# rlorenzo/facet

Hardware: AMD Instinct MI355X
Metric: images/sec whole-node (TOPIQ+SAMP+CLIP+InsightFace ensemble), 1024² batch (higher is better)
Workload: dtype f32

## Files before the change

### facet_amd/csrc/engine.hip

```cpp
#include "engine.h"
#include "onnx_graph.h"
#include "wino64_maps.h"
#include <algorithm>
#include <cmath>
#include <cstdlib>

namespace fe {

void WeightStore::set(const std::string& name, const float* data, const int64_t* shape, int ndim) {
  HostTensor h;
  h.shape.assign(shape, shape + ndim);
  h.data.assign(data, data + h.numel());
  t_[name] = std::move(h);
}
const HostTensor& WeightStore::get(const std::string& name) const {
  auto it = t_.find(name);
  if (it == t_.end()) throw Error("missing weight tensor '" + name + "'");
  return it->second;
}

float* DeviceWeights::upload(const std::vector<float>& v) {
  void* p = nullptr;
  const size_t b = v.size() * sizeof(float);
  FE_HIP(hipMalloc(&p, b ? b : 16));
// ... 219 lines not shown
  p.w = w.w; p.scale = w.scale; p.shift = w.shift; p.slope = w.slope;
  FE_CHECK(o.act != ACT_PRELU || w.slope, "conv: PReLU without slopes");
  if (o.res) {
    FE_CHECK(o.res->c == y.c && o.res->pixels() == y.pixels(), "conv: residual shape mismatch");
    p.res = o.res->p; p.ldr = o.res->ld;
  }
  if (o.gate) {
    FE_CHECK(o.gate->pixels() == y.pixels() && (o.gate->c == 1 || o.gate->c == y.c), "conv: gate shape mismatch");
    p.gate = o.gate->p; p.ldg = o.gate->ld; p.gate_c1 = o.gate->c == 1;
  }
  p.y = y.p; p.ldy = y.ld;
  p.N = x.n; p.H = x.h; p.W = x.w; p.Cin = w.CinPad;
  p.Ho = y.h; p.Wo = y.w; p.Cout = w.Cout;
  p.KH = w.KH; p.KW = w.KW; p.sh = o.sh; p.sw = o.sw; p.ph = o.ph; p.pw = o.pw; p.dh = o.dh; p.dw = o.dw;
  FE_CHECK(y.h == conv_out_dim(x.h, w.KH, o.sh, o.ph, o.dh) && y.w == conv_out_dim(x.w, w.KW, o.sw, o.pw, o.dw),
           "conv: output dims %dx%d inconsistent with input %dx%d", y.h, y.w, x.h, x.w);
  p.K = w.K; p.Kp = w.Kp;
  p.M = (int)y.pixels();
  FE_CHECK(y.pixels() < (1ull << 31), "conv: M too large");
  p.act = o.act; p.res_after_act = o.res_after_act;
  p.variant = c.force_variant;
  if (w.wtap && o.act != ACT_PRELU && o.sh == 1 && o.sw == 1 && !o.res && !o.gate && p.variant == 0 && y.h == x.h && y.w == x.w) {
    const int T = w.KH * w.KW * w.Cout, Tp = (T + 3) & ~3;
    const size_t mark = c.arena.mark();
    Tensor z = c.arena.tensor(x.n, x.h, x.w, Tp);
    ConvParams q{};
    q.x = x.p; q.ldx = x.ld; q.w = w.wtap; q.y = z.p; q.ldy = Tp;
    q.N = x.n; q.H = x.h; q.W = x.w; q.Cin = w.CinPad; q.Ho = x.h; q.Wo = x.w; q.Cout = T;
    q.KH = q.KW = 1; q.sh = q.sw = q.dh = q.dw = 1;
    q.K = w.CinPad; q.Kp = w.KpT; q.M = (int)x.pixels();
    launch_conv(q, c.stream);
    launch_tap_gather(z.p, Tp, x.n, x.h, x.w, w.KH, w.KW, o.ph, o.pw, o.dh, o.dw, w.Cout, w.scale, w.shift, o.act, y.p,
                      y.ld, y.h, y.w, c.stream);
    c.arena.rewind(mark);
    c.flops_accum += 2.0 * p.M * (double)(w.KH * w.KW * w.Cin) * (w.CoutAlg ? w.CoutAlg : p.Cout);
    return;
  }
  static const bool no_wino = getenv("FE_NO_WINO") != nullptr;
  const bool wino_plain = !o.res && (o.act == ACT_NONE || o.act == ACT_RELU);
  if (w.wino && !no_wino && p.variant == 0 && o.sh == 1 && o.sw == 1 && o.ph == 1 && o.pw == 1 && o.dh == 1 && o.dw == 1 &&
      !o.gate && (wino_plain || (w.wino_m == 4 && (o.act == ACT_NONE || o.act == ACT_RELU || o.act == ACT_PRELU))) && y.h == x.h && y.w == x.w && (((uintptr_t)x.p | (uintptr_t)y.p) & 15) == 0 &&
      x.ld % 4 == 0 && y.ld % 4 == 0) {
    const int ts = w.wino_m, planes = (ts + 2) * (ts + 2);
    const int th = (x.h + ts - 1) / ts, tw = (x.w + ts - 1) / ts;
    const size_t tiles = (size_t)x.n * th * tw;
    const size_t wino_bytes = (size_t)planes * tiles * ((size_t)w.CinPad + w.Cout) * sizeof(float) + 1024;
    if (tiles < (1u << 30) / 36 && c.arena.mark() + wino_bytes <= c.arena.capacity()) {
      const size_t mark = c.arena.mark();
      float* V = (float*)c.arena.alloc((size_t)planes * tiles * w.CinPad * sizeof(float));
      float* Mb = (float*)c.arena.alloc((size_t)planes * tiles * w.Cout * sizeof(float));
      hipEvent_t e0 = nullptr, e1 = nullptr;
      if (c.profile) {
        FE_HIP(hipEventCreate(&e0)); FE_HIP(hipEventCreate(&e1));
        FE_HIP(hipEventRecord(e0, c.stream));
      }
      if (ts == 2) launch_wino_input(x, th, tw, V, c.stream);
      else launch_wino4_input(x, th, tw, V, c.stream);
      ConvParams g{};
      g.x = V; g.ldx = w.CinPad; g.w = w.wino; g.ldw = w.CinPad; g.y = Mb; g.ldy = w.Cout;
      g.M = (int)tiles; g.K = w.CinPad; g.Cout = w.Cout;
      g.N = 1; g.H = 1; g.W = g.M; g.Ho = 1; g.Wo = g.M; g.KH = g.KW = 1; g.sh = g.sw = g.dh = g.dw = 1;
      g.Kp = w.CinPad; g.Cin = w.CinPad;
      g.batch = planes; g.nb1 = 1; g.xs2 = (long long)tiles * w.CinPad; g.ws2 = (long long)w.Cout * w.CinPad; g.ys2 = (long long)tiles * w.Cout;
      launch_conv(g, c.stream);
      if (ts == 2) launch_wino_output(Mb, y, th, tw, w.scale, w.shift, o.act == ACT_RELU, c.stream);
      else launch_wino4_output(Mb, y, th, tw, w.scale, w.shift, o.act, w.slope, o.res, o.res_after_act, c.stream);
      if (c.profile) {
        FE_HIP(hipEventRecord(e1, c.stream));
        FE_HIP(hipEventSynchronize(e1));
        float ms = 0.f;
        FE_HIP(hipEventElapsedTime(&ms, e0, e1));
        (void)hipEventDestroy(e0); (void)hipEventDestroy(e1);
        char nm[128];
        snprintf(nm, sizeof nm, "wino3x3 M=%d K=%d N=%d", p.M, p.K, p.Cout);
        c.timings.push_back({nm, 2.0 * p.M * (double)(9 * w.Cin) * p.Cout, 0.0, ms});
      }
      c.arena.rewind(mark);
      c.flops_accum += 2.0 * p.M * (double)(w.KH * w.KW * w.Cin) * (w.CoutAlg ? w.CoutAlg : p.Cout);
      c.flops_saved += 2.0 * p.M * (double)(9 * w.Cin) * (w.CoutAlg ? w.CoutAlg : p.Cout) - 2.0 * (double)planes * (double)tiles * w.CinPad * w.Cout;
      return;
    }
  }
  static const bool no_wino64 = getenv("FE_NO_WINO64") != nullptr;
  if (w.wino64 && !no_wino64 && p.variant == 0 && (o.act == ACT_NONE || o.act == ACT_RELU || o.act == ACT_PRELU) && o.sh == 1 && o.sw == 1 && o.ph == 1 && o.pw == 1 && o.dh == 1 && o.dw == 1 && !o.gate && y.h == x.h &&
      y.w == x.w && (((uintptr_t)x.p | (uintptr_t)y.p | (uintptr_t)(o.res ? o.res->p : nullptr)) & 15) == 0 && x.ld % 4 == 0 && y.ld % 4 == 0 &&
      (!o.res || o.res->ld % 4 == 0) && (unsigned long long)x.h * x.w * x.ld * 4ull < 0xF0000000ull) {
    hipEvent_t e0 = nullptr, e1 = nullptr;
    if (c.profile) {
      FE_HIP(hipEventCreate(&e0)); FE_HIP(hipEventCreate(&e1));
      FE_HIP(hipEventRecord(e0, c.stream));
    }
    launch_wino64(x, y, w.wino64, w.scale, w.shift, w.slope, o.act, o.res, o.res_after_act, c.stream);
    const double direct = 2.0 * p.M * (double)(9 * w.Cin) * (w.CoutAlg ? w.CoutAlg : p.Cout);
    if (c.profile) {
      FE_HIP(hipEventRecord(e1, c.stream));
      FE_HIP(hipEventSynchronize(e1));
      float ms = 0.f;
      FE_HIP(hipEventElapsedTime(&ms, e0, e1));
      (void)hipEventDestroy(e0); (void)hipEventDestroy(e1);
      char nm[128];
      snprintf(nm, sizeof nm, "wino64 3x3 M=%d K=%d N=%d", p.M, p.K, p.Cout);
      const double bytes = 4.0 * ((double)x.pixels() * x.c + (double)y.pixels() * y.c * (o.res ? 2 : 1) + (double)w64::U_FLOATS);
      c.timings.push_back({nm, direct, bytes, ms});
    }
    const double tiles = (double)x.n * ((x.h + 1) / 2) * ((x.w + 1) / 2);
    c.flops_accum += direct;
    c.flops_saved += direct - 2.0 * 16.0 * tiles * 64.0 * w.Cout;
    return;
  }
  static const bool no_splitk = getenv("FE_NO_SPLITK") != nullptr;
  static const int splitk_min = getenv("FE_SPLITK_MIN") ? atoi(getenv("FE_SPLITK_MIN")) : 2048;
  if (!no_splitk && w.KH == 1 && w.KW == 1 && o.sh == 1 && o.sw == 1 && o.ph == 0 && o.pw == 0 && !o.gate && p.variant == 0 && p.M <= 256 &&
      w.CinPad >= splitk_min && w.K == w.CinPad && (size_t)((p.M + 127) / 128) * ((w.Cout + 63) / 64) < 64 &&
      (o.act == ACT_NONE || o.act == ACT_RELU || o.act == ACT_PRELU)) {
    int splits = 0;
    for (int s = 64; s >= 2; --s)
      if (w.CinPad % s == 0 && (w.CinPad / s) % 32 == 0 && w.CinPad / s >= 256) { splits = s; break; }
    const size_t part_bytes = (size_t)splits * p.M * w.Cout * sizeof(float);
    if (splits && c.arena.mark() + part_bytes + 1024 <= c.arena.capacity()) {
      const size_t mark = c.arena.mark();
      float* part = (float*)c.arena.alloc(part_bytes);
      const int Ks = w.CinPad / splits;
      hipEvent_t e0 = nullptr, e1 = nullptr;
      if (c.profile) {
        FE_HIP(hipEventCreate(&e0)); FE_HIP(hipEventCreate(&e1));
        FE_HIP(hipEventRecord(e0, c.stream));
      }
      ConvParams g{};
      g.x = x.p; g.ldx = x.ld; g.w = w.w; g.ldw = w.Kp; g.y = part; g.ldy = w.Cout;
      g.M = p.M; g.K = Ks; g.Kp = Ks; g.Cin = Ks; g.Cout = w.Cout;
      g.N = 1; g.H = 1; g.W = g.M; g.Ho = 1; g.Wo = g.M; g.KH = g.KW = 1; g.sh = g.sw = g.dh = g.dw = 1;
      g.batch = splits; g.nb1 = 1; g.xs2 = Ks; g.ws2 = Ks; g.ys2 = (long long)p.M * w.Cout;
      launch_conv(g, c.stream);
      launch_splitk_reduce(part, splits, p.M, w.Cout, w.scale, w.shift, w.slope, o.act, o.res ? o.res->p : nullptr, o.res ? o.res->ld : 0,
                           o.res_after_act, y.p, y.ld, c.stream);
      if (c.profile) {
        FE_HIP(hipEventRecord(e1, c.stream));
        FE_HIP(hipEventSynchronize(e1));
        float ms = 0.f;
        FE_HIP(hipEventElapsedTime(&ms, e0, e1));
        (void)hipEventDestroy(e0); (void)hipEventDestroy(e1);
        char nm[128];
        snprintf(nm, sizeof nm, "splitk%d 1x1 M=%d K=%d N=%d", splits, p.M, p.K, p.Cout);
        c.timings.push_back({nm, 2.0 * p.M * (double)w.Cin * (w.CoutAlg ? w.CoutAlg : p.Cout), 0.0, ms});
      }
      c.arena.rewind(mark);
      c.flops_accum += 2.0 * p.M * (double)w.Cin * (w.CoutAlg ? w.CoutAlg : p.Cout);
      return;
    }
  }
  static const bool no_stem = getenv("FE_NO_STEM") != nullptr;
  const bool stem = w.wstem && !no_stem && p.variant == 0 && o.sh == o.sw && o.ph == w.KH / 2 && o.pw == w.KW / 2 && o.dh == 1 && o.dw == 1 && !o.res &&
                    !o.gate && (o.act == ACT_NONE || o.act == ACT_RELU || o.act == ACT_PRELU);
  auto launch = [&]() {
    if (stem && launch_stem(x.p, x.ld, x.n, x.h, x.w, w.wstem, w.scale, w.shift, w.slope, w.Cout, w.KH, o.sh,
                            o.act == ACT_RELU ? 1 : (o.act == ACT_PRELU ? 2 : 0), y.p, y.ld, y.h, y.w, c.stream))
      return;
    launch_conv(p, c.stream);
  };
  if (c.profile) {
    hipEvent_t e0, e1;
    FE_HIP(hipEventCreate(&e0)); FE_HIP(hipEventCreate(&e1));
    FE_HIP(hipEventRecord(e0, c.stream));
    launch();
    FE_HIP(hipEventRecord(e1, c.stream));
    FE_HIP(hipEventSynchronize(e1));
    float ms = 0.f;
    FE_HIP(hipEventElapsedTime(&ms, e0, e1));
    (void)hipEventDestroy(e0); (void)hipEventDestroy(e1);
// ... 475 lines not shown
```

### facet_amd/csrc/fe_common.h

```cpp
#pragma once
#include <hip/hip_runtime.h>
#include "fe_check.h"
#include <cstdint>
#include <cstdio>
#include <atomic>
#include <cstring>
#include <map>
#include <mutex>
#include <stdexcept>
#include <string>
#include <vector>

namespace fe {


#define FE_HIP(expr)                                                                      \
  do {                                                                                    \
    hipError_t _e = (expr);                                                               \
    if (_e != hipSuccess) {                                                               \
      char _b[512];                                                                       \
      snprintf(_b, sizeof _b, "%s:%d: %s -> %s", __FILE__, __LINE__, #expr,               \
               hipGetErrorString(_e));                                                    \
      throw fe::Error(_b);                                                                \
    }                                                                                     \
// ... 175 lines not shown
  size_t cap_ = 0, off_ = 0, high_ = 0;
};

template <class T>
struct ConvParamsT {
  const T* x; int ldx;
  const T* w;
  const float* scale;
  const float* shift;
  const float* slope;
  const T* res; int ldr;
  const T* gate; int ldg;
  T* y; int ldy;
  int N, H, W, Cin, Ho, Wo, Cout;
  int KH, KW, sh, sw, ph, pw, dh, dw;
  int K, Kp, M;
  int act;
  int res_after_act;
  int gate_c1;
  int vec_epi;
  int unit_stride;
  int ldw;
  int batch, nb1;
  long long xs1, xs2, ws1, ws2, ys1, ys2, hs1;
  int buf_ok; unsigned x_span, w_span;
  unsigned y_span, r_span, g_span;
  int variant;
  int cb;
  int pad_store;
  const float* res32; int ldr32;
  float* y32; int ldy32;
  unsigned r32_span, y32_span;
  int a_wrap;
  int split_lo_off;
  int exact_act;
};
using ConvParams = ConvParamsT<float>;
using ConvParamsH = ConvParamsT<bf16>;

struct ConvW {
  float* w = nullptr;
  float* scale = nullptr;
  float* shift = nullptr;
  float* slope = nullptr;
  int Cout = 0, Cin = 0, CinPad = 0, KH = 1, KW = 1, K = 0, Kp = 0;
  int CoutAlg = 0;
  float* wtap = nullptr;
  int wino_m = 0;
  float* wino = nullptr;
  float* wino64 = nullptr;
  float* wstem = nullptr;
  float* wn16 = nullptr;
  int KpT = 0;
  void* wh = nullptr;
  int hprec = 0;
  int KpH = 0, cb = 0, CinPadH = 0;
  void* wtap_h = nullptr;
  int KpTH = 0;
  uint8_t* w8 = nullptr;
  float* w8_scale = nullptr;
};

template <class T>
struct ConvOptsT {
  int sh = 1, sw = 1, ph = 0, pw = 0, dh = 1, dw = 1;
  int act = ACT_NONE;
  const TensorT<T>* res = nullptr;
  int res_after_act = 0;
  const TensorT<T>* gate = nullptr;
  const TensorT<float>* res32 = nullptr;
  const TensorT<float>* y32 = nullptr;
};
using ConvOpts = ConvOptsT<float>;

constexpr int CONV_KALIGN = 32;
constexpr int CONV_KALIGN_H = 64;

void launch_conv(const ConvParams& p, hipStream_t s);
void launch_wino_input(const Tensor& x, int th, int tw, float* V, hipStream_t s);
void launch_wino_output(const float* Mb, const Tensor& y, int th, int tw, const float* scale, const float* shift, int relu, hipStream_t s);
void launch_wino4_input(const Tensor& x, int th, int tw, float* V, hipStream_t s);
void launch_wino4_output(const float* Mb, const Tensor& y, int th, int tw, const float* scale, const float* shift, int act, const float* slope,
                         const Tensor* res, int res_after_act, hipStream_t s);
void launch_wino64(const Tensor& x, const Tensor& y, const float* U, const float* scale, const float* shift, const float* slope, int act,
                   const Tensor* res, int res_after_act, hipStream_t s);
template <class TO>
bool launch_stem(const float* x, int ldx, int N, int H, int W, const float* wstem, const float* scale, const float* shift, const float* slope,
                 int Cout, int k, int stride, int act, TO* y, int ldy, int Ho, int Wo, hipStream_t s);
void launch_conv_narrow(const ConvParams& p, hipStream_t s);
void launch_conv_dma(const ConvParams& p, int tile, hipStream_t s);
void launch_conv_bf16(const ConvParamsH& p, hipStream_t s);
void launch_conv_bf16(const ConvParamsT<f16>& p, hipStream_t s);
template <class T, class Launch>
inline bool conv_split_by_images(const ConvParamsT<T>& p, Launch&& launch) {
  if (p.batch > 1 || p.N <= 1 || (long long)p.N * p.Ho * p.Wo != (long long)p.M) return false;
  const unsigned long long in_img = (unsigned long long)p.H * p.W * p.ldx * sizeof(T);
  unsigned long long out_img = (unsigned long long)p.Ho * p.Wo * (unsigned long long)(p.ldy > p.ldr ? p.ldy : p.ldr) * sizeof(T);
  const unsigned long long out32_img = (unsigned long long)p.Ho * p.Wo * (unsigned long long)(p.ldy32 > p.ldr32 ? p.ldy32 : p.ldr32) * sizeof(float);
  if ((p.y32 || p.res32) && out32_img > out_img) out_img = out32_img;
  const unsigned long long per_img = in_img > out_img ? in_img : out_img;
  constexpr unsigned long long LIMIT = 0xF0000000ull;
  if (per_img >= LIMIT) return false;
  const int ng = (int)(LIMIT / per_img);
  if (ng >= p.N) return false;
  for (int i0 = 0; i0 < p.N; i0 += ng) {
    ConvParamsT<T> q = p;
    const int n = ng < p.N - i0 ? ng : p.N - i0;
    const size_t opix = (size_t)i0 * p.Ho * p.Wo;
    q.N = n; q.M = n * p.Ho * p.Wo;
    q.x = p.x + (size_t)i0 * p.H * p.W * p.ldx;
    if (p.y) q.y = p.y + opix * p.ldy;
    if (p.y32) q.y32 = p.y32 + opix * p.ldy32;
    if (p.res32) q.res32 = p.res32 + opix * p.ldr32;
    if (p.res) q.res = p.res + opix * p.ldr;
    if (p.gate) q.gate = p.gate + opix * p.ldg;
    launch(q);
  }
  return true;
}

double conv_flops(const ConvParams& p);

void launch_u8_to_nhwc4_norm(const uint8_t* src, float* dst, size_t pixels, const float mean[3],
                             const float stdv[3], int bgr, hipStream_t s);
template <class T> void launch_nchw_to_nhwc(const float* src, T* dst, int n, int c, int h, int w, int cpad, hipStream_t s);
template <class T> void launch_nhwc_to_nchw(const T* src, int lds_, float* dst, int n, int c, int h, int w, hipStream_t s);
template <class T> void launch_maxpool(const TensorT<T>& x, const TensorT<T>& y, int k, int stride, int pad, hipStream_t s);
template <class T> void launch_bilinear(const TensorT<T>& x, const TensorT<T>& y, hipStream_t s);
template <class T> void launch_adaptive_avgpool(const TensorT<T>& x, const TensorT<T>& y, hipStream_t s);
void launch_convert(const float* x, bf16* y, size_t n, hipStream_t s);
void launch_convert(const bf16* x, float* y, size_t n, hipStream_t s);
void launch_convert(const float* x, f16* y, size_t n, hipStream_t s);
void launch_convert(const f16* x, float* y, size_t n, hipStream_t s);
void launch_splitk_reduce(const float* part, int splits, int M, int N, const float* scale, const float* shift, const float* slope, int act,
                          const float* res, int ldr, int res_after_act, float* y, int ldy, hipStream_t s);
template <class T>
void launch_tap_gather(const T* z, int ldz, int n, int h, int w, int kh, int kw, int ph, int pw, int dh, int dw,
                       int cout, const float* scale, const float* shift, int act, T* y, int ldy, int ho, int wo,
                       hipStream_t s);
void launch_attention(const float* q, int ldq, const float* k, int ldk, const float* vt, int lp, const float* bv, float* o,
                      int ldo, int B, int H, int Lq, int Lk, int dmodel, int causal, hipStream_t s);
void launch_attention(const bf16* q, int ldq, const bf16* k, int ldk, const bf16* vt, int lp, const float* bv, bf16* o,
                      int ldo, int B, int H, int Lq, int Lk, int dmodel, int causal, hipStream_t s);
void launch_attention(const f16* q, int ldq, const f16* k, int ldk, const f16* vt, int lp, const float* bv, f16* o,
                      int ldo, int B, int H, int Lq, int Lk, int dmodel, int causal, hipStream_t s);
void launch_attention_split(const f16* q, const f16* k, int ld, int lo_off, const f16* vt_hi, const f16* vt_lo, int lp, f16* o, int ldo, int o_lo_off,
                            int B, int H, int Lq, int Lk, int dmodel, hipStream_t s);
template <class TI, class TW, class TO>
void launch_gemm_skinny(const TI* x, int ldx, const TW* w, int ldw, const float* scale, const float* shift, TO* y,
                        int ldy, int M, int N, int K, int act, hipStream_t s);
void launch_sigmoid(const Tensor& x, const Tensor& y, hipStream_t s);
void launch_add(const Tensor& a, const Tensor& b, const Tensor& y, hipStream_t s);
void launch_layernorm_split(const float* x, int ldx, f16* y, int ldy, const float* g, const float* b, int rows, int d, float eps, hipStream_t s);
void launch_split_hi_lo(const float* x, f16* y, size_t rows, int cols, hipStream_t s);
template <class T, class TO>
void launch_layernorm(const T* x, int ldx, TO* y, int ldy, const float* g, const float* b,
                      int rows, int d, float eps, hipStream_t s);
void launch_softmax_rows(float* x, int ld, int rows, int d, hipStream_t s);
void launch_softmax_rows_pad(float* x, int ld, int rows, int d, hipStream_t s);
template <class T>
void launch_add_rows_bcast(T* y, int ldy, const float* pos, int rows, int L, int d, hipStream_t s);

void launch_affine_act(const Tensor& x, const Tensor& y, const float* scale, const float* shift, int act, const float* slope,
                       hipStream_t s);
void launch_binary(const Tensor& a, const Tensor& b, const Tensor& y, int op, int act, hipStream_t s);
void launch_gather_strided(const float* src, float* dst, const long long dims[6], const long long sstr[6], hipStream_t s);
// ... 51 lines not shown
```

### facet_amd/csrc/kernels_wino64.hip

```cpp
#include "fe_common.h"
#include "wino64_maps.h"

namespace fe {

struct W64Params {
  const float* x; int ldx, cin;
  int N, H, W;
  float* y; int ldy, cout;
  const float* U;
  const float *scale, *shift, *slope;
  const float* res; int ldr;
  int res_after_act;
  int bx, by, nblocks;
};

constexpr int W64_PATCH_FLOATS = w64::CHUNK_UNITS * 2;

template <int A>
__global__ __launch_bounds__(256, 1) __attribute__((amdgpu_waves_per_eu(1, 1))) void wino64_kernel(const W64Params p) {
  using namespace w64;
  __shared__ __attribute__((aligned(16))) float sP[2 * W64_PATCH_FLOATS];
  const int t = threadIdx.x, lane = t & 63, wave = __builtin_amdgcn_readfirstlane(t >> 6);
  const int tg = wave & 1, half = wave >> 1;
  const int tl = lane & 31, kk = lane >> 5;
  const int ty = tile_y(tg, tl), tx = tile_x(tl);
  constexpr int act = A;

  int pc_py[PIECES_PER_THREAD], pc_px[PIECES_PER_THREAD], pc_dst[PIECES_PER_THREAD];
#pragma unroll
  for (int i = 0; i < PIECES_PER_THREAD; ++i) {
    const int idx = t + 256 * i, pixel = idx / PARTS, part = idx % PARTS;
    pc_py[i] = pixel / PATCH; pc_px[i] = pixel - pc_py[i] * PATCH;
    pc_dst[i] = idx < PIECES ? 2 * patch_unit(2 * part, pc_py[i], pc_px[i]) : -1;
  }
  const int part4 = (t % PARTS) * 4;
  auto block_origin = [&](const int v, int& b, int& y0, int& x0) {
    const int per = p.bx * p.by;
    b = v / per;
    const int rem = v - b * per, byi = rem / p.bx;
    y0 = byi * BLOCK; x0 = (rem - byi * p.bx) * BLOCK;
  };
  fe_v4f pf[PIECES_PER_THREAD];
  typedef unsigned w64_v4u __attribute__((ext_vector_type(4)));
  constexpr unsigned OOB = 0xFFFFFFF0u;
  const unsigned img_bytes = (unsigned)p.H * (unsigned)p.W * (unsigned)p.ldx * 4u;
  auto fetch_stage = [&](const int v, const int c) __attribute__((always_inline)) {
    const bool live = v < p.nblocks;
    int b, y0, x0;
    block_origin(live ? v : 0, b, y0, x0);
    const __amdgpu_buffer_rsrc_t rs = __builtin_amdgcn_make_buffer_rsrc(const_cast<float*>(p.x + (size_t)b * p.H * p.W * p.ldx), 0, (int)img_bytes, 0x00020000);
    const bool ch_in = live && c * CHUNK_CH + part4 < p.cin;
#pragma unroll
    for (int i = 0; i < PIECES_PER_THREAD; ++i) {
      const int gy = y0 - 1 + pc_py[i], gx = x0 - 1 + pc_px[i];
      const bool in = pc_dst[i] >= 0 && ch_in && (unsigned)gy < (unsigned)p.H && (unsigned)gx < (unsigned)p.W;
      const unsigned off = in ? ((unsigned)(gy * p.W + gx) * (unsigned)p.ldx + (unsigned)(c * CHUNK_CH + part4)) * 4u : OOB;
      pf[i] = __builtin_bit_cast(fe_v4f, (w64_v4u)__builtin_amdgcn_raw_buffer_load_b128(rs, (int)off, 0, 0));
    }
  };
  auto store_stage = [&](const int buf) __attribute__((always_inline)) {
    float* const pd = sP + buf * W64_PATCH_FLOATS;
#pragma unroll
    for (int i = 0; i < PIECES_PER_THREAD; ++i)
      if (pc_dst[i] >= 0) {
        *reinterpret_cast<float2*>(pd + pc_dst[i]) = make_float2(pf[i].x, pf[i].y);
        *reinterpret_cast<float2*>(pd + pc_dst[i] + 2 * PAIR_UNITS) = make_float2(pf[i].z, pf[i].w);
      }
  };

  const float* const ubase = p.U + u_index(0, half, 0, lane, 0);
  fe_v4f ua[STEPS_PER_CHUNK][4];
  auto fetch_u = [&](const int step, fe_v4f (&u)[4]) __attribute__((always_inline)) {
#pragma unroll
    for (int q = 0; q < 4; ++q) u[q] = *reinterpret_cast<const fe_v4f*>(ubase + step * U_STEP_FLOATS + q * 256);
  };
#pragma unroll
  for (int s0 = 0; s0 < STEPS_PER_CHUNK; ++s0) fetch_u(s0, ua[s0]);
  fetch_stage(blockIdx.x, 0);
  store_stage(0);
  __syncthreads();

  const int lane_unit = patch_unit(kk, 2 * ty, 2 * tx);
  for (int v = blockIdx.x; v < p.nblocks; v += gridDim.x) {
    fe_f32x16 acc[16];
#pragma unroll
    for (int pl = 0; pl < 16; ++pl)
#pragma unroll
      for (int e = 0; e < 16; ++e) acc[pl][e] = 0.f;

#pragma unroll 1
    for (int c = 0; c < NCHUNK; ++c) {
      if (c + 1 < NCHUNK) fetch_stage(v, c + 1);
      else fetch_stage(v + (int)gridDim.x, 0);
      const float* const buf = sP + (c & 1) * W64_PATCH_FLOATS + 2 * lane_unit;
      float2 dq[2][16];
      auto read_pair = [&](const int j, float2 (&d)[16]) __attribute__((always_inline)) {
#pragma unroll
        for (int dy = 0; dy < 4; ++dy)
#pragma unroll
          for (int dx = 0; dx < 4; ++dx)
            d[4 * dy + dx] = *reinterpret_cast<const float2*>(buf + 2 * (2 * j * PAIR_UNITS + dy * ROW_UNITS + (dx & 1) * (ROW_UNITS / 2) + (dx >> 1)));
      };
      const int nstage = ((c + 1) & (NCHUNK - 1)) * STEPS_PER_CHUNK;
      read_pair(0, dq[0]);
#pragma unroll
      for (int j = 0; j < STEPS_PER_CHUNK / 2; ++j) {
        if (j + 1 < STEPS_PER_CHUNK / 2) read_pair(j + 1, dq[(j + 1) & 1]);
        __builtin_amdgcn_sched_barrier(0);
#pragma unroll
        for (int s2 = 0; s2 < 2; ++s2) {
          float d[16], vv[16];
#pragma unroll
          for (int i = 0; i < 16; ++i) d[i] = s2 ? dq[j & 1][i].y : dq[j & 1][i].x;
          input_transform(d, vv);
#pragma unroll
          for (int pl = 0; pl < 16; ++pl) acc[pl] = __builtin_amdgcn_mfma_f32_32x32x2f32(ua[2 * j + s2][pl >> 2][pl & 3], vv[pl], acc[pl], 0, 0, 0);
          __builtin_amdgcn_sched_barrier(0);
          fetch_u(nstage + 2 * j + s2, ua[2 * j + s2]);
        }
      }
      store_stage((c + 1) & 1);
      __syncthreads();
    }

    int b, y0, x0;
    block_origin(v, b, y0, x0);
    const int oy = y0 + 2 * ty, ox = x0 + 2 * tx;
    size_t pix[4]; bool ok[4];
#pragma unroll
    for (int i = 0; i < 4; ++i) {
      const int yy = oy + (i >> 1), xx = ox + (i & 1);
      ok[i] = yy < p.H && xx < p.W;
      pix[i] = ok[i] ? ((size_t)b * p.H + yy) * p.W + xx : 0;
    }
    float4 scv[4], sfv[4], slv[4];
#pragma unroll
    for (int g = 0; g < 4; ++g) {
      const int cb = acc_channel(half, lane, 4 * g), cl = cb < p.cout ? cb : 0;
      scv[g] = p.scale ? *reinterpret_cast<const float4*>(p.scale + cl) : make_float4(1.f, 1.f, 1.f, 1.f);
      sfv[g] = p.shift ? *reinterpret_cast<const float4*>(p.shift + cl) : make_float4(0.f, 0.f, 0.f, 0.f);
      slv[g] = act == ACT_PRELU ? *reinterpret_cast<const float4*>(p.slope + cl) : make_float4(0.f, 0.f, 0.f, 0.f);
    }
#pragma unroll
    for (int g = 0; g < 4; ++g) {
      const int cb = acc_channel(half, lane, 4 * g);
      if (cb >= p.cout) continue;
      float o[4][4];
#pragma unroll
      for (int e = 0; e < 4; ++e) {
        float m[16], yq[4];
#pragma unroll
        for (int pl = 0; pl < 16; ++pl) m[pl] = acc[pl][4 * g + e];
        output_transform(m, yq);
#pragma unroll
        for (int i = 0; i < 4; ++i) o[i][e] = yq[i];
      }
      const float4 sc = scv[g], sf = sfv[g], sl = slv[g];
#pragma unroll
      for (int i = 0; i < 4; ++i) {
        if (!ok[i]) continue;
        float4 r = make_float4(0.f, 0.f, 0.f, 0.f);
        if (p.res) r = *reinterpret_cast<const float4*>(p.res + pix[i] * p.ldr + cb);
        float4 q;
        q.x = o[i][0] * sc.x + sf.x; q.y = o[i][1] * sc.y + sf.y; q.z = o[i][2] * sc.z + sf.z; q.w = o[i][3] * sc.w + sf.w;
        if (p.res && !p.res_after_act) { q.x += r.x; q.y += r.y; q.z += r.z; q.w += r.w; }
        if (act == ACT_PRELU) {
          q.x = q.x > 0.f ? q.x : q.x * sl.x; q.y = q.y > 0.f ? q.y : q.y * sl.y;
          q.z = q.z > 0.f ? q.z : q.z * sl.z; q.w = q.w > 0.f ? q.w : q.w * sl.w;
        } else {
          q.x = fe_apply_act(q.x, act); q.y = fe_apply_act(q.y, act); q.z = fe_apply_act(q.z, act); q.w = fe_apply_act(q.w, act);
        }
        if (p.res && p.res_after_act) { q.x += r.x; q.y += r.y; q.z += r.z; q.w += r.w; }
        *reinterpret_cast<float4*>(p.y + pix[i] * p.ldy + cb) = q;
      }
    }
  }
}

void launch_wino64(const Tensor& x, const Tensor& y, const float* U, const float* scale, const float* shift, const float* slope, int act,
                   const Tensor* res, int res_after_act, hipStream_t s) {
  FE_CHECK(x.c > 0 && x.c <= 64 && x.c % 4 == 0 && y.c > 0 && y.c <= 64 && y.c % 4 == 0 && y.n == x.n && y.h == x.h && y.w == x.w, "wino64: %dx%dx%d -> %dx%dx%d", x.h,
           x.w, x.c, y.h, y.w, y.c);
  FE_CHECK(x.ld % 4 == 0 && y.ld % 4 == 0 && (((uintptr_t)x.p | (uintptr_t)y.p | (uintptr_t)U) & 15) == 0, "wino64: operands must be 16-byte aligned");
  FE_CHECK(!res || (res->ld % 4 == 0 && ((uintptr_t)res->p & 15) == 0 && res->c == y.c && res->pixels() == y.pixels()), "wino64: residual view");
  FE_CHECK(act == ACT_NONE || act == ACT_RELU || (act == ACT_PRELU && slope), "wino64: activation %d (PReLU needs slopes)", act);
  FE_CHECK((unsigned long long)x.h * x.w * x.ld * 4ull < 0xF0000000ull, "wino64: one image must stay below 4 GiB (32-bit buffer offsets)");
  W64Params p{};
  p.x = x.p; p.ldx = x.ld; p.cin = x.c; p.N = x.n; p.H = x.h; p.W = x.w;
  p.y = y.p; p.ldy = y.ld; p.cout = y.c;
  p.U = U; p.scale = scale; p.shift = shift; p.slope = slope;
  p.res = res ? res->p : nullptr; p.ldr = res ? res->ld : 0;
  p.res_after_act = res_after_act;
  p.bx = (x.w + w64::BLOCK - 1) / w64::BLOCK; p.by = (x.h + w64::BLOCK - 1) / w64::BLOCK;
  const long long nb = (long long)x.n * p.bx * p.by;
  FE_CHECK(nb < (1ll << 30), "wino64: too many blocks");
  p.nblocks = (int)nb;
  const int grid = p.nblocks < 256 ? p.nblocks : 256;
  if (act == ACT_NONE) hipLaunchKernelGGL(wino64_kernel<ACT_NONE>, dim3(grid), dim3(256), 0, s, p);
  else if (act == ACT_RELU) hipLaunchKernelGGL(wino64_kernel<ACT_RELU>, dim3(grid), dim3(256), 0, s, p);
  else hipLaunchKernelGGL(wino64_kernel<ACT_PRELU>, dim3(grid), dim3(256), 0, s, p);
  FE_HIP(hipGetLastError());
}

}
```

### facet_amd/csrc/wino64_maps.h

```cpp
#pragma once

#if defined(__HIPCC__)
#define W64_HD __host__ __device__ __forceinline__
#else
#define W64_HD inline
#endif

namespace fe {
namespace w64 {

constexpr int BLOCK = 16;
constexpr int PATCH = BLOCK + 2;
constexpr int CHUNK_CH = 8;
constexpr int NCHUNK = 64 / CHUNK_CH;
constexpr int STEPS_PER_CHUNK = CHUNK_CH / 2;
constexpr int NSTEPS = NCHUNK * STEPS_PER_CHUNK;
constexpr int ROW_UNITS = 20;
constexpr int PAIR_UNITS = PATCH * ROW_UNITS;
constexpr int CHUNK_UNITS = (CHUNK_CH / 2) * PAIR_UNITS;
constexpr int PARTS = CHUNK_CH / 4;
constexpr int PIECES = PATCH * PATCH * PARTS;
constexpr int PIECES_PER_THREAD = (PIECES + 255) / 256;
constexpr int U_STEP_FLOATS = 2 * 4 * 64 * 4;
constexpr int U_FLOATS = NSTEPS * U_STEP_FLOATS;

W64_HD int tile_y(int tg, int tl) { return 4 * tg + (tl >> 3); }
W64_HD int tile_x(int tl) { return tl & 7; }
W64_HD int channel(int step, int k) { return 4 * (step >> 1) + 2 * k + (step & 1); }
W64_HD int acc_channel(int half, int lane, int e) { return half * 32 + 8 * (e >> 2) + 4 * (lane >> 5) + (e & 3); }
W64_HD int u_index(int step, int half, int q, int lane, int j) { return ((((step * 2 + half) * 4 + q) * 64 + lane) << 2) + j; }
W64_HD int patch_unit(int pair, int py, int px) { return pair * PAIR_UNITS + py * ROW_UNITS + (px & 1) * (ROW_UNITS / 2) + (px >> 1); }

W64_HD void input_transform(const float d[16], float v[16]) {
  float t[16];
  for (int c = 0; c < 4; ++c) {
    t[0 + c] = d[0 + c] - d[8 + c];
    t[4 + c] = d[4 + c] + d[8 + c];
    t[8 + c] = d[8 + c] - d[4 + c];
    t[12 + c] = d[4 + c] - d[12 + c];
  }
  for (int a = 0; a < 4; ++a) {
    v[4 * a + 0] = t[4 * a + 0] - t[4 * a + 2];
    v[4 * a + 1] = t[4 * a + 1] + t[4 * a + 2];
    v[4 * a + 2] = t[4 * a + 2] - t[4 * a + 1];
    v[4 * a + 3] = t[4 * a + 1] - t[4 * a + 3];
  }
}
W64_HD void output_transform(const float m[16], float y[4]) {
  float s[8];
  for (int b = 0; b < 4; ++b) {
    s[b] = (m[b] + m[4 + b]) + m[8 + b];
    s[4 + b] = (m[4 + b] - m[8 + b]) - m[12 + b];
  }
  for (int i = 0; i < 2; ++i) {
    y[2 * i + 0] = (s[4 * i + 0] + s[4 * i + 1]) + s[4 * i + 2];
    y[2 * i + 1] = (s[4 * i + 1] - s[4 * i + 2]) - s[4 * i + 3];
  }
}

inline void pack_u(const float* w, int Cout, int Cin, float* U) {
  static const double G[4][3] = {{1, 0, 0}, {0.5, 0.5, 0.5}, {0.5, -0.5, 0.5}, {0, 0, 1}};
  for (int i = 0; i < U_FLOATS; ++i) U[i] = 0.f;
  for (int step = 0; step < NSTEPS; ++step)
    for (int half = 0; half < 2; ++half)
      for (int lane = 0; lane < 64; ++lane) {
        const int co = half * 32 + (lane & 31), ci = channel(step, lane >> 5);
        if (co >= Cout || ci >= Cin) continue;
        const float* g = w + ((long long)co * Cin + ci) * 9;
        double tmp[4][3];
        for (int a = 0; a < 4; ++a)
          for (int q = 0; q < 3; ++q) tmp[a][q] = G[a][0] * g[q] + G[a][1] * g[3 + q] + G[a][2] * g[6 + q];
        for (int a = 0; a < 4; ++a)
          for (int b = 0; b < 4; ++b) {
            const double u = tmp[a][0] * G[b][0] + tmp[a][1] * G[b][1] + tmp[a][2] * G[b][2];
            U[u_index(step, half, a, lane, b)] = (float)u;
          }
      }
}

}
}
```

Measured before the change: 234.6.

## Defer wino64 epilogue through LDS and overlap it with next block's MFMAs

```diff
diff --git a/facet_amd/csrc/engine.hip b/facet_amd/csrc/engine.hip
--- a/facet_amd/csrc/engine.hip
+++ b/facet_amd/csrc/engine.hip
@@ -325,9 +325,12 @@
     }
   }
   static const bool no_wino64 = getenv("FE_NO_WINO64") != nullptr;
-  if (w.wino64 && !no_wino64 && p.variant == 0 && (o.act == ACT_NONE || o.act == ACT_RELU || o.act == ACT_PRELU) && o.sh == 1 && o.sw == 1 && o.ph == 1 && o.pw == 1 && o.dh == 1 && o.dw == 1 && !o.gate && y.h == x.h &&
+  const long long w64_blocks = (long long)x.n * ((x.h + w64::BLOCK - 1) / w64::BLOCK) * ((x.w + w64::BLOCK - 1) / w64::BLOCK);
+  const bool w64_act = o.act == ACT_NONE || o.act == ACT_RELU || o.act == ACT_PRELU || ((o.act == ACT_GELU || o.act == ACT_SIGMOID) && w64_blocks > W64_MAX_GRID);
+  const unsigned long long w64_ld = std::max(std::max(x.ld, y.ld), o.res ? o.res->ld : 0);
+  if (w.wino64 && !no_wino64 && p.variant == 0 && w64_act && o.sh == 1 && o.sw == 1 && o.ph == 1 && o.pw == 1 && o.dh == 1 && o.dw == 1 && !o.gate && y.h == x.h &&
       y.w == x.w && (((uintptr_t)x.p | (uintptr_t)y.p | (uintptr_t)(o.res ? o.res->p : nullptr)) & 15) == 0 && x.ld % 4 == 0 && y.ld % 4 == 0 &&
-      (!o.res || o.res->ld % 4 == 0) && (unsigned long long)x.h * x.w * x.ld * 4ull < 0xF0000000ull) {
+      (!o.res || o.res->ld % 4 == 0) && (unsigned long long)x.h * x.w * w64_ld * 4ull < 0xF0000000ull) {
     hipEvent_t e0 = nullptr, e1 = nullptr;
     if (c.profile) {
       FE_HIP(hipEventCreate(&e0)); FE_HIP(hipEventCreate(&e1));
diff --git a/facet_amd/csrc/fe_common.h b/facet_amd/csrc/fe_common.h
--- a/facet_amd/csrc/fe_common.h
+++ b/facet_amd/csrc/fe_common.h
@@ -281,6 +281,7 @@
 void launch_wino4_input(const Tensor& x, int th, int tw, float* V, hipStream_t s);
 void launch_wino4_output(const float* Mb, const Tensor& y, int th, int tw, const float* scale, const float* shift, int act, const float* slope,
                          const Tensor* res, int res_after_act, hipStream_t s);
+constexpr int W64_MAX_GRID = 256;
 void launch_wino64(const Tensor& x, const Tensor& y, const float* U, const float* scale, const float* shift, const float* slope, int act,
                    const Tensor* res, int res_after_act, hipStream_t s);
 template <class TO>
diff --git a/facet_amd/csrc/kernels_wino64.hip b/facet_amd/csrc/kernels_wino64.hip
--- a/facet_amd/csrc/kernels_wino64.hip
+++ b/facet_amd/csrc/kernels_wino64.hip
@@ -20,6 +20,8 @@
 __global__ __launch_bounds__(256, 1) __attribute__((amdgpu_waves_per_eu(1, 1))) void wino64_kernel(const W64Params p) {
   using namespace w64;
   __shared__ __attribute__((aligned(16))) float sP[2 * W64_PATCH_FLOATS];
+  __shared__ __attribute__((aligned(16))) float sImg[IMAGE_FLOATS];
+  __shared__ __attribute__((aligned(16))) float sEpi[3 * 64];
   const int t = threadIdx.x, lane = t & 63, wave = __builtin_amdgcn_readfirstlane(t >> 6);
   const int tg = wave & 1, half = wave >> 1;
   const int tl = lane & 31, kk = lane >> 5;
@@ -78,10 +80,63 @@
   for (int s0 = 0; s0 < STEPS_PER_CHUNK; ++s0) fetch_u(s0, ua[s0]);
   fetch_stage(blockIdx.x, 0);
   store_stage(0);
+  if (t < 64) {
+    const int cl = t < p.cout ? t : 0;
+    sEpi[t] = p.scale ? p.scale[cl] : 1.f;
+    sEpi[64 + t] = p.shift ? p.shift[cl] : 0.f;
+    sEpi[128 + t] = act == ACT_PRELU ? p.slope[cl] : 0.f;
+  }
   __syncthreads();
 
+  const unsigned y_bytes = (unsigned)p.H * (unsigned)p.W * (unsigned)p.ldy * 4u, r_bytes = (unsigned)p.H * (unsigned)p.W * (unsigned)p.ldr * 4u;
+  __amdgpu_buffer_rsrc_t d_ry, d_rr;
+  int d_y0 = 0, d_x0 = 0;
+  auto drain_block = [&](const int u) __attribute__((always_inline)) {
+    int b;
+    block_origin(u < 0 ? 0 : u, b, d_y0, d_x0);
+    const size_t img = (size_t)b * p.H * p.W;
+    d_ry = __builtin_amdgcn_make_buffer_rsrc(p.y + img * p.ldy, 0, u < 0 ? 0 : (int)y_bytes, 0x00020000);
+    d_rr = __builtin_amdgcn_make_buffer_rsrc(const_cast<float*>(p.res ? p.res + img * p.ldr : p.y), 0, u < 0 || !p.res ? 0 : (int)r_bytes, 0x00020000);
+  };
+  auto drain_off = [&](const int k, const int ld) __attribute__((always_inline)) {
+    const int yy = d_y0 + k, xx = d_x0 + (t >> 4), cb = drain_channel(t);
+    return yy < p.H && xx < p.W && cb < p.cout ? ((unsigned)(yy * p.W + xx) * (unsigned)ld + (unsigned)cb) * 4u : OOB;
+  };
+  fe_v4f d_res = {0.f, 0.f, 0.f, 0.f};
+  float d_q[4];
+  float4 d_sc, d_sf, d_sl = make_float4(0.f, 0.f, 0.f, 0.f);
+  auto drain_fetch_res = [&](const int k) __attribute__((always_inline)) {
+    d_res = __builtin_bit_cast(fe_v4f, (w64_v4u)__builtin_amdgcn_raw_buffer_load_b128(d_rr, (int)drain_off(k, p.ldr), 0, 0));
+  };
+  auto drain_read = [&](const int k) __attribute__((always_inline)) {
+    const int cb = drain_channel(t);
+    const float4 raw = *reinterpret_cast<const float4*>(sImg + image_index(drain_pixel(k, t), cb));
+    d_q[0] = raw.x; d_q[1] = raw.y; d_q[2] = raw.z; d_q[3] = raw.w;
+    d_sc = *reinterpret_cast<const float4*>(sEpi + cb);
+    d_sf = *reinterpret_cast<const float4*>(sEpi + 64 + cb);
+    if (act == ACT_PRELU) d_sl = *reinterpret_cast<const float4*>(sEpi + 128 + cb);
+  };
+  const bool res_before = p.res && !p.res_after_act, res_after = p.res && p.res_after_act;
+  auto drain_affine = [&]() __attribute__((always_inline)) {
+    d_q[0] = d_q[0] * d_sc.x + d_sf.x; d_q[1] = d_q[1] * d_sc.y + d_sf.y; d_q[2] = d_q[2] * d_sc.z + d_sf.z; d_q[3] = d_q[3] * d_sc.w + d_sf.w;
+#pragma unroll
+    for (int e = 0; e < 4; ++e) d_q[e] = res_before ? d_q[e] + d_res[e] : d_q[e];
+  };
+  auto drain_act = [&](const int e) __attribute__((always_inline)) {
+    float q = d_q[e];
+    if (act == ACT_PRELU) q = q > 0.f ? q : q * (e == 0 ? d_sl.x : e == 1 ? d_sl.y : e == 2 ? d_sl.z : d_sl.w);
+    else q = fe_apply_act(q, act);
+    d_q[e] = res_after ? q + d_res[e] : q;
+  };
+  auto drain_store = [&](const int k) __attribute__((always_inline)) {
+    const fe_v4f q = {d_q[0], d_q[1], d_q[2], d_q[3]};
+    __builtin_amdgcn_raw_buffer_store_b128(__builtin_bit_cast(w64_v4u, q), d_ry, (int)drain_off(k, p.ldy), 0, 0);
+  };
+
   const int lane_unit = patch_unit(kk, 2 * ty, 2 * tx);
+  int vlast = -1;
   for (int v = blockIdx.x; v < p.nblocks; v += gridDim.x) {
+    drain_block(vlast);
     fe_f32x16 acc[16];
 #pragma unroll
     for (int pl = 0; pl < 16; ++pl)
@@ -90,6 +145,7 @@
 
 #pragma unroll 1
     for (int c = 0; c < NCHUNK; ++c) {
+      if (p.res) drain_fetch_res(DRAIN_ROWS_PER_STAGE * c);
       if (c + 1 < NCHUNK) fetch_stage(v, c + 1);
       else fetch_stage(v + (int)gridDim.x, 0);
       const float* const buf = sP + (c & 1) * W64_PATCH_FLOATS + 2 * lane_unit;
@@ -113,8 +169,20 @@
 #pragma unroll
           for (int i = 0; i < 16; ++i) d[i] = s2 ? dq[j & 1][i].y : dq[j & 1][i].x;
           input_transform(d, vv);
-#pragma unroll
-          for (int pl = 0; pl < 16; ++pl) acc[pl] = __builtin_amdgcn_mfma_f32_32x32x2f32(ua[2 * j + s2][pl >> 2][pl & 3], vv[pl], acc[pl], 0, 0, 0);
+          const int krow = DRAIN_ROWS_PER_STAGE * c + j;
+          if (s2 == 0 && j > 0 && p.res) drain_fetch_res(krow);
+#pragma unroll
+          for (int pl = 0; pl < 16; ++pl) {
+            acc[pl] = __builtin_amdgcn_mfma_f32_32x32x2f32(ua[2 * j + s2][pl >> 2][pl & 3], vv[pl], acc[pl], 0, 0, 0);
+            if (s2 == 1 && (pl == 1 || (pl >= 4 && pl <= 9))) {
+              __builtin_amdgcn_sched_barrier(0);
+              if (pl == 1) drain_read(krow);
+              else if (pl == 4) drain_affine();
+              else if (pl < 9) drain_act(pl - 5);
+              else drain_store(krow);
+              __builtin_amdgcn_sched_barrier(0);
+            }
+          }
           __builtin_amdgcn_sched_barrier(0);
           fetch_u(nstage + 2 * j + s2, ua[2 * j + s2]);
         }
@@ -123,28 +191,9 @@
       __syncthreads();
     }
 
-    int b, y0, x0;
-    block_origin(v, b, y0, x0);
-    const int oy = y0 + 2 * ty, ox = x0 + 2 * tx;
-    size_t pix[4]; bool ok[4];
-#pragma unroll
-    for (int i = 0; i < 4; ++i) {
-      const int yy = oy + (i >> 1), xx = ox + (i & 1);
-      ok[i] = yy < p.H && xx < p.W;
-      pix[i] = ok[i] ? ((size_t)b * p.H + yy) * p.W + xx : 0;
-    }
-    float4 scv[4], sfv[4], slv[4];
-#pragma unroll
-    for (int g = 0; g < 4; ++g) {
-      const int cb = acc_channel(half, lane, 4 * g), cl = cb < p.cout ? cb : 0;
-      scv[g] = p.scale ? *reinterpret_cast<const float4*>(p.scale + cl) : make_float4(1.f, 1.f, 1.f, 1.f);
-      sfv[g] = p.shift ? *reinterpret_cast<const float4*>(p.shift + cl) : make_float4(0.f, 0.f, 0.f, 0.f);
-      slv[g] = act == ACT_PRELU ? *reinterpret_cast<const float4*>(p.slope + cl) : make_float4(0.f, 0.f, 0.f, 0.f);
-    }
 #pragma unroll
     for (int g = 0; g < 4; ++g) {
       const int cb = acc_channel(half, lane, 4 * g);
-      if (cb >= p.cout) continue;
       float o[4][4];
 #pragma unroll
       for (int e = 0; e < 4; ++e) {
@@ -155,23 +204,31 @@
 #pragma unroll
         for (int i = 0; i < 4; ++i) o[i][e] = yq[i];
       }
-      const float4 sc = scv[g], sf = sfv[g], sl = slv[g];
-#pragma unroll
-      for (int i = 0; i < 4; ++i) {
-        if (!ok[i]) continue;
-        float4 r = make_float4(0.f, 0.f, 0.f, 0.f);
-        if (p.res) r = *reinterpret_cast<const float4*>(p.res + pix[i] * p.ldr + cb);
-        float4 q;
-        q.x = o[i][0] * sc.x + sf.x; q.y = o[i][1] * sc.y + sf.y; q.z = o[i][2] * sc.z + sf.z; q.w = o[i][3] * sc.w + sf.w;
-        if (p.res && !p.res_after_act) { q.x += r.x; q.y += r.y; q.z += r.z; q.w += r.w; }
-        if (act == ACT_PRELU) {
-          q.x = q.x > 0.f ? q.x : q.x * sl.x; q.y = q.y > 0.f ? q.y : q.y * sl.y;
-          q.z = q.z > 0.f ? q.z : q.z * sl.z; q.w = q.w > 0.f ? q.w : q.w * sl.w;
-        } else {
-          q.x = fe_apply_act(q.x, act); q.y = fe_apply_act(q.y, act); q.z = fe_apply_act(q.z, act); q.w = fe_apply_act(q.w, act);
-        }
-        if (p.res && p.res_after_act) { q.x += r.x; q.y += r.y; q.z += r.z; q.w += r.w; }
-        *reinterpret_cast<float4*>(p.y + pix[i] * p.ldy + cb) = q;
+#pragma unroll
+      for (int i = 0; i < 4; ++i)
+        *reinterpret_cast<float4*>(sImg + image_index((2 * ty + (i >> 1)) * BLOCK + 2 * tx + (i & 1), cb)) = make_float4(o[i][0], o[i][1], o[i][2], o[i][3]);
+    }
+    __syncthreads();
+    vlast = v;
+  }
+
+  if (vlast >= 0) {
+    drain_block(vlast);
+    for (int k0 = 0; k0 < BLOCK; k0 += 8) {
+      fe_v4f r8[8];
+#pragma unroll
+      for (int i = 0; i < 8; ++i) {
+        if (p.res) drain_fetch_res(k0 + i);
+        r8[i] = d_res;
+      }
+#pragma unroll
+      for (int i = 0; i < 8; ++i) {
+        d_res = r8[i];
+        drain_read(k0 + i);
+        drain_affine();
+#pragma unroll
+        for (int e = 0; e < 4; ++e) drain_act(e);
+        drain_store(k0 + i);
       }
     }
   }
@@ -183,8 +240,9 @@
            x.w, x.c, y.h, y.w, y.c);
   FE_CHECK(x.ld % 4 == 0 && y.ld % 4 == 0 && (((uintptr_t)x.p | (uintptr_t)y.p | (uintptr_t)U) & 15) == 0, "wino64: operands must be 16-byte aligned");
   FE_CHECK(!res || (res->ld % 4 == 0 && ((uintptr_t)res->p & 15) == 0 && res->c == y.c && res->pixels() == y.pixels()), "wino64: residual view");
-  FE_CHECK(act == ACT_NONE || act == ACT_RELU || (act == ACT_PRELU && slope), "wino64: activation %d (PReLU needs slopes)", act);
-  FE_CHECK((unsigned long long)x.h * x.w * x.ld * 4ull < 0xF0000000ull, "wino64: one image must stay below 4 GiB (32-bit buffer offsets)");
+  FE_CHECK(act == ACT_NONE || act == ACT_RELU || act == ACT_GELU || act == ACT_SIGMOID || (act == ACT_PRELU && slope), "wino64: activation %d (PReLU needs slopes)", act);
+  const unsigned long long ldmax = std::max(std::max(x.ld, y.ld), res ? res->ld : 0);
+  FE_CHECK((unsigned long long)x.h * x.w * ldmax * 4ull < 0xF0000000ull, "wino64: one image must stay below 4 GiB (32-bit buffer offsets)");
   W64Params p{};
   p.x = x.p; p.ldx = x.ld; p.cin = x.c; p.N = x.n; p.H = x.h; p.W = x.w;
   p.y = y.p; p.ldy = y.ld; p.cout = y.c;
@@ -195,9 +253,11 @@
   const long long nb = (long long)x.n * p.bx * p.by;
   FE_CHECK(nb < (1ll << 30), "wino64: too many blocks");
   p.nblocks = (int)nb;
-  const int grid = p.nblocks < 256 ? p.nblocks : 256;
+  const int grid = p.nblocks < W64_MAX_GRID ? p.nblocks : W64_MAX_GRID;
   if (act == ACT_NONE) hipLaunchKernelGGL(wino64_kernel<ACT_NONE>, dim3(grid), dim3(256), 0, s, p);
   else if (act == ACT_RELU) hipLaunchKernelGGL(wino64_kernel<ACT_RELU>, dim3(grid), dim3(256), 0, s, p);
+  else if (act == ACT_GELU) hipLaunchKernelGGL(wino64_kernel<ACT_GELU>, dim3(grid), dim3(256), 0, s, p);
+  else if (act == ACT_SIGMOID) hipLaunchKernelGGL(wino64_kernel<ACT_SIGMOID>, dim3(grid), dim3(256), 0, s, p);
   else hipLaunchKernelGGL(wino64_kernel<ACT_PRELU>, dim3(grid), dim3(256), 0, s, p);
   FE_HIP(hipGetLastError());
 }
diff --git a/facet_amd/csrc/wino64_maps.h b/facet_amd/csrc/wino64_maps.h
--- a/facet_amd/csrc/wino64_maps.h
+++ b/facet_amd/csrc/wino64_maps.h
@@ -30,6 +30,12 @@
 W64_HD int acc_channel(int half, int lane, int e) { return half * 32 + 8 * (e >> 2) + 4 * (lane >> 5) + (e & 3); }
 W64_HD int u_index(int step, int half, int q, int lane, int j) { return ((((step * 2 + half) * 4 + q) * 64 + lane) << 2) + j; }
 W64_HD int patch_unit(int pair, int py, int px) { return pair * PAIR_UNITS + py * ROW_UNITS + (px & 1) * (ROW_UNITS / 2) + (px >> 1); }
+
+constexpr int IMAGE_FLOATS = BLOCK * BLOCK * 64;
+constexpr int DRAIN_ROWS_PER_STAGE = BLOCK / NCHUNK;
+W64_HD int image_index(int pixel, int ch) { return pixel * 64 + (((ch >> 2) ^ ((pixel >> 1) & 7)) << 2) + (ch & 3); }
+W64_HD int drain_pixel(int k, int t) { return k * BLOCK + (t >> 4); }
+W64_HD int drain_channel(int t) { return (t & 15) * 4; }
 
 W64_HD void input_transform(const float d[16], float v[16]) {
   float t[16];
```

After: 236.6 (median of 6 runs). About the same (+0.9%).
